# edwardyehuang/iSeg

Hardware: AMD Instinct MI355X
Metric: train_images_per_sec (ConvNeXt-T+ASPP 512x512 crop, fwd+bwd+AdamW, whole job) (higher is better)
Workload: dtype bf16

## Files before the change

include/iseg_hip.h:

```cpp
#ifndef ISEG_HIP_H
#define ISEG_HIP_H

#include <stddef.h>
#include <stdint.h>

#ifdef __cplusplus
extern "C" {
#endif

#ifndef ISEG_HIP_STREAM_T
#define ISEG_HIP_STREAM_T
typedef struct ihipStream_t* iseg_stream_t;
#endif

#define ISEG_STATUS_OK 0
#define ISEG_STATUS_ARG (-1)
#define ISEG_STATUS_HIP (-2)
#define ISEG_STATUS_UNSUPPORTED (-3)
#define ISEG_STATUS_WORKSPACE (-4)

#define ISEG_DTYPE_F32 0
#define ISEG_DTYPE_BF16 1

#define ISEG_ACT_NONE 0
// ... 46 lines not shown
int iseg_gemm_splits(const iseg_gemm_args* args_h);
int iseg_gemm_slabs(const iseg_gemm_args* args_h);
int iseg_gemm_variant(const iseg_gemm_args* args_h);
size_t iseg_gemm_workspace_bytes(const iseg_gemm_args* args_h);
int iseg_gemm(const iseg_gemm_args* args_h, void* ws, size_t ws_bytes, iseg_stream_t stream);
int iseg_gemm_reduce(const iseg_gemm_args* args_h, void* ws, size_t ws_bytes, iseg_stream_t stream);
int iseg_gemm_tn_pair_splits(const iseg_gemm_args* g0, const iseg_gemm_args* g1);
int iseg_gemm_tn_pair(const iseg_gemm_args* g0, void* ws0, size_t ws0_bytes, const iseg_gemm_args* g1, void* ws1, size_t ws1_bytes,
                      iseg_stream_t stream);

int iseg_layernorm_fwd(const void* x, const float* gamma, const float* beta, void* y, float* mean, float* rstd, int64_t rows,
                       int C, float eps, int dtype, iseg_stream_t stream);
size_t iseg_layernorm_bwd_workspace_bytes(int64_t rows, int C);
int iseg_layernorm_bwd(const void* dy, const void* x, const float* gamma, const float* mean, const float* rstd, void* dx,
                       const void* dx_add, float* dgamma, float* dbeta, int accumulate_param_grads, int64_t rows, int C,
                       int dtype, void* ws, size_t ws_bytes, iseg_stream_t stream);
int iseg_layernorm_post_fwd(const void* x, const float* gamma, const float* beta, const float* colscale, const float* rowscale,
                            int64_t rows_per_group, const void* residual, void* y, float* mean, float* rstd, int64_t rows, int C, float eps,
                            int dtype, iseg_stream_t stream);
int iseg_layernorm_post_bwd(const void* dy, const void* x, const float* gamma, const float* beta, const float* colscale, const float* rowscale,
                            int64_t rows_per_group, const float* mean, const float* rstd, void* dx, float* dgamma, float* dbeta,
                            float* dcolscale, int64_t rows, int C, int dtype, void* ws, size_t ws_bytes, iseg_stream_t stream);
int iseg_layernorm_gather_fwd(const void* x, const int32_t* src_index, const float* gamma, const float* beta, void* y, float* mean,
                              float* rstd, int64_t rows_out, int C, float eps, int dtype, iseg_stream_t stream);
int iseg_layernorm_gather_bwd(const void* dy, const int32_t* dy_index, const void* x, const float* gamma, const float* mean,
                              const float* rstd, void* dx, const void* dx_add, float* dgamma, float* dbeta, int accumulate_param_grads,
                              int64_t rows, int C, int dtype, void* ws, size_t ws_bytes, iseg_stream_t stream);

int iseg_dwconv2d_fwd(const void* x, const float* w, const float* bias, const void* add, void* y, int N, int H, int W, int C,
                      int K, int dil, int pad_t, int pad_l, int flip, int dtype, iseg_stream_t stream);
int iseg_dwconv2d7_mfma(const void* x, const float* w, const float* bias, const void* add, void* y, int N, int H, int W, int C, int pad_t,
                        int pad_l, int flip, iseg_stream_t stream);
size_t iseg_dwconv2d_bwd_weight_workspace_bytes(int N, int H, int W, int C, int K);
int iseg_dwconv2d_bwd_weight(const void* x, const void* dy, float* dw, float* db, int accumulate, int N, int H, int W, int C,
                             int K, int dil, int pad_t, int pad_l, int dtype, void* ws, size_t ws_bytes, iseg_stream_t stream);

int iseg_dwconv2d_strided_fwd(const void* x, const float* w, const float* bias, void* y, int N, int H, int W, int C, int K, int stride, int dil,
                              int pad_t, int pad_l, int Ho, int Wo, int dtype, iseg_stream_t stream);
int iseg_dwconv2d_strided_bwd_data(const void* dy, const float* w, void* dx, int N, int H, int W, int C, int K, int stride, int dil, int pad_t,
                                   int pad_l, int Ho, int Wo, int dtype, iseg_stream_t stream);
size_t iseg_dwconv2d_strided_bwd_weight_workspace_bytes(int N, int Ho, int Wo, int C, int K);
int iseg_dwconv2d_strided_bwd_weight(const void* x, const void* dy, float* dw, float* db, int accumulate, int N, int H, int W, int C, int K,
                                     int stride, int dil, int pad_t, int pad_l, int Ho, int Wo, int dtype, void* ws, size_t ws_bytes,
                                     iseg_stream_t stream);

size_t iseg_bn_workspace_bytes(int64_t rows, int C);
int iseg_bn_stats(const void* x, int64_t ldx, float* packed, int64_t rows, int C, int dtype, void* ws, size_t ws_bytes,
                  iseg_stream_t stream);
int iseg_bn_finalize(const float* packed, int C, float eps, float momentum, float* mean, float* rstd, float* moving_mean,
                     float* moving_var, iseg_stream_t stream);
int iseg_bn_apply_fwd(const void* x, int64_t ldx, const float* mean, const float* rstd, const float* gamma, const float* beta,
                      void* y, int64_t ldy, int64_t rows, int C, int relu, int dtype, iseg_stream_t stream);
int iseg_bn_apply_fwd_packed(const void* x, int64_t ldx, const float* packed, float eps, float momentum, const float* gamma, const float* beta,
                             float* mean, float* rstd, float* moving_mean, float* moving_var, void* y, int64_t ldy, int64_t rows, int C,
                             int relu, int dtype, iseg_stream_t stream);
int iseg_bn_bwd_reduce(const void* dy, int64_t lddy, const void* x, int64_t ldx, const void* y, int64_t ldy, const float* mean,
                       const float* rstd, float* sums, int64_t rows, int C, int relu, int dtype, void* ws, size_t ws_bytes,
                       iseg_stream_t stream);
int iseg_bn_bwd_apply(const void* dy, int64_t lddy, const void* x, int64_t ldx, const void* y, int64_t ldy, const float* mean,
                      const float* rstd, const float* gamma, const float* sums, float inv_n, void* dx, int64_t lddx, int64_t rows,
                      int C, int relu, int dtype, iseg_stream_t stream);
int iseg_bn_bwd_apply_acc(const void* dy, int64_t lddy, const void* x, int64_t ldx, const void* y, int64_t ldy, const float* mean,
                          const float* rstd, const float* gamma, const float* sums, float inv_n, void* dx, int64_t lddx, float* dgamma,
                          float* dbeta, int64_t rows, int C, int relu, int dtype, iseg_stream_t stream);
int iseg_bn_bwd_reduce_remask(const void* dy, int64_t lddy, const void* x, int64_t ldx, const float* mean, const float* rstd,
                              const float* gamma, const float* beta, float* sums, int64_t rows, int C, int dtype, void* ws, size_t ws_bytes,
// ... 348 lines not shown
```

iseg_amd/_hip.py:

```python
import ctypes as C
import os

_HERE = os.path.dirname(os.path.abspath(__file__))
LIB_PATH = os.path.join(_HERE, "lib", "libiseg_hip.so")

F32, BF16 = 0, 1
ACT_NONE, ACT_RELU, ACT_GELU, ACT_GELU_GRAD, ACT_RELU_GRAD, ACT_MUL_AUX, ACT_SIGMOID, ACT_SWISH = 0, 1, 2, 3, 4, 5, 6, 7


class HipLibraryMissing(RuntimeError):
    pass


class HipCallError(RuntimeError):
    pass


class GemmArgs(C.Structure):
    _fields_ = [
        ("A", C.c_void_p), ("lda", C.c_int64), ("a_kcontig", C.c_int),
        ("B", C.c_void_p), ("ldb", C.c_int64), ("b_kcontig", C.c_int),
        ("D", C.c_void_p), ("ldd", C.c_int64),
        ("M", C.c_int64), ("N", C.c_int64), ("K", C.c_int64),
        ("in_dtype", C.c_int), ("out_dtype", C.c_int),
# ... 16 lines not shown
    _fields_ = [(n, C.c_int) for n in ("N", "H", "W", "Cin", "Cout", "KH", "KW", "sh", "sw", "dh", "dw", "pt", "pl", "Ho", "Wo", "groups")]


_p, _i, _l, _f, _z, _u64 = C.c_void_p, C.c_int, C.c_int64, C.c_float, C.c_size_t, C.c_uint64

SIGNATURES = {
    "iseg_version": (_i, []),
    "iseg_last_error": (_z, [C.c_char_p, _z]),
    "iseg_gemm_splits": (_i, [C.POINTER(GemmArgs)]),
    "iseg_gemm_tn_pair_splits": (_i, [C.POINTER(GemmArgs), C.POINTER(GemmArgs)]),
    "iseg_gemm_tn_pair": (_i, [C.POINTER(GemmArgs), _p, _z, C.POINTER(GemmArgs), _p, _z, _p]),
    "iseg_gemm_slabs": (_i, [C.POINTER(GemmArgs)]),
    "iseg_gemm_variant": (_i, [C.POINTER(GemmArgs)]),
    "iseg_gemm_workspace_bytes": (_z, [C.POINTER(GemmArgs)]),
    "iseg_gemm": (_i, [C.POINTER(GemmArgs), _p, _z, _p]),
    "iseg_gemm_reduce": (_i, [C.POINTER(GemmArgs), _p, _z, _p]),
    "iseg_layernorm_fwd": (_i, [_p, _p, _p, _p, _p, _p, _l, _i, _f, _i, _p]),
    "iseg_layernorm_bwd_workspace_bytes": (_z, [_l, _i]),
    "iseg_layernorm_bwd": (_i, [_p, _p, _p, _p, _p, _p, _p, _p, _p, _i, _l, _i, _i, _p, _z, _p]),
    "iseg_layernorm_post_fwd": (_i, [_p, _p, _p, _p, _p, _l, _p, _p, _p, _p, _l, _i, _f, _i, _p]),
    "iseg_layernorm_post_bwd": (_i, [_p, _p, _p, _p, _p, _p, _l, _p, _p, _p, _p, _p, _p, _l, _i, _i, _p, _z, _p]),
    "iseg_layernorm_gather_fwd": (_i, [_p, _p, _p, _p, _p, _p, _p, _l, _i, _f, _i, _p]),
    "iseg_layernorm_gather_bwd": (_i, [_p, _p, _p, _p, _p, _p, _p, _p, _p, _p, _i, _l, _i, _i, _p, _z, _p]),
    "iseg_dwconv2d_fwd": (_i, [_p, _p, _p, _p, _p, _i, _i, _i, _i, _i, _i, _i, _i, _i, _i, _p]),
    "iseg_dcnv2_sample_fwd": (_i, [_p, _p, _p, _i, _i, _i, _i, _i, _p]),
    "iseg_dcnv2_sample_bwd_workspace_bytes": (_z, [_i, _i, _i, _i]),
    "iseg_dcnv2_sample_bwd": (_i, [_p, _p, _p, _p, _p, _i, _i, _i, _i, _i, _p, _z, _p]),
    "iseg_qkv_rope": (_i, [_p, _p, _p, _p, _p, _l, _i, _i, _i, _i, _i, _i, _p]),
    "iseg_glu_fwd": (_i, [_p, _l, _p, _l, _p, _l, _l, _i, _i, _i, _p]),
    "iseg_glu_bwd": (_i, [_p, _l, _p, _l, _p, _l, _p, _l, _p, _l, _l, _i, _i, _i, _p]),
    "iseg_dwconv2d7_mfma": (_i, [_p, _p, _p, _p, _p, _i, _i, _i, _i, _i, _i, _i, _p]),
    "iseg_dwconv2d_bwd_weight_workspace_bytes": (_z, [_i, _i, _i, _i, _i]),
    "iseg_dwconv2d_bwd_weight": (_i, [_p, _p, _p, _p, _i, _i, _i, _i, _i, _i, _i, _i, _i, _i, _p, _z, _p]),
    "iseg_dwconv2d_strided_fwd": (_i, [_p, _p, _p, _p, _i, _i, _i, _i, _i, _i, _i, _i, _i, _i, _i, _i, _p]),
    "iseg_dwconv2d_strided_bwd_data": (_i, [_p, _p, _p, _i, _i, _i, _i, _i, _i, _i, _i, _i, _i, _i, _i, _p]),
    "iseg_dwconv2d_strided_bwd_weight_workspace_bytes": (_z, [_i, _i, _i, _i, _i]),
    "iseg_dwconv2d_strided_bwd_weight": (_i, [_p, _p, _p, _p, _i, _i, _i, _i, _i, _i, _i, _i, _i, _i, _i, _i, _i, _p, _z, _p]),
    "iseg_dcn_center_blend_fwd": (_i, [_p, _p, _p, _p, _l, _i, _i, _i, _p]),
    "iseg_dcn_center_blend_bwd": (_i, [_p, _p, _p, _p, _p, _p, _p, _l, _i, _i, _i, _p]),
    "iseg_bn_workspace_bytes": (_z, [_l, _i]),
    "iseg_bn_stats": (_i, [_p, _l, _p, _l, _i, _i, _p, _z, _p]),
    "iseg_bn_finalize": (_i, [_p, _i, _f, _f, _p, _p, _p, _p, _p]),
    "iseg_bn_apply_fwd": (_i, [_p, _l, _p, _p, _p, _p, _p, _l, _l, _i, _i, _i, _p]),
    "iseg_bn_apply_fwd_packed": (_i, [_p, _l, _p, _f, _f, _p, _p, _p, _p, _p, _p, _p, _l, _l, _i, _i, _i, _p]),
    "iseg_bn_bwd_reduce": (_i, [_p, _l, _p, _l, _p, _l, _p, _p, _p, _l, _i, _i, _i, _p, _z, _p]),
    "iseg_bn_bwd_apply": (_i, [_p, _l, _p, _l, _p, _l, _p, _p, _p, _p, _f, _p, _l, _l, _i, _i, _i, _p]),
    "iseg_bn_bwd_apply_acc": (_i, [_p, _l, _p, _l, _p, _l, _p, _p, _p, _p, _f, _p, _l, _p, _p, _l, _i, _i, _i, _p]),
    "iseg_bn_bwd_reduce_remask": (_i, [_p, _l, _p, _l, _p, _p, _p, _p, _p, _l, _i, _i, _p, _z, _p]),
    "iseg_bn_bwd_apply_remask": (_i, [_p, _l, _p, _l, _p, _p, _p, _p, _p, _f, _p, _l, _p, _p, _l, _i, _i, _p]),
    "iseg_bn_relu_upsample_add": (_i, [_p, _p, _p, _p, _p, _p, _p, _i, _i, _i, _i, _i, _i, _i, _p]),
    "iseg_rsqrt_eps": (_i, [_p, _f, _p, _i, _p]),
    "iseg_mbconv_supported": (_i, [_i, _i, _i, _i]),
    "iseg_mbconv_partials_bytes": (_z, [_i, _i, _i, _i]),
    "iseg_se_excite_bwd_workspace_bytes": (_z, [_i, _i, _i]),
    "iseg_bn_swish_se_squeeze": (_i, [_p, _p, _p, _p, _p, _p, _z, _i, _i, _i, _i, _p]),
    "iseg_se_excite_fwd": (_i, [_p, _i, _i, _i, _i, _p, _p, _p, _p, _p, _p, _p, _p]),
    "iseg_bn_swish_gate_fwd": (_i, [_p, _p, _p, _p, _p, _p, _p, _i, _i, _i, _i, _p]),
    "iseg_bn_swish_gate_bwd_reduce": (_i, [_p, _p, _p, _p, _p, _p, _p, _z, _i, _i, _i, _i, _p]),
    "iseg_se_excite_bwd": (_i, [_p, _i, _i, _i, _i, _p, _p, _p, _p, _p, _p, _p, _p, _p, _i, _p, _p, _p, _z, _p]),
    "iseg_bn_swish_gate_bwd_apply": (_i, [_p, _p, _p, _p, _p, _p, _p, _p, _p, _f, _i, _p, _p, _p, _i, _i, _i, _i, _p]),
    "iseg_sepconv_supported": (_i, [_i, _i, _i, _i, _i, _i, _i]),
    "iseg_relu_dwconv3_stats_workspace_bytes": (_z, [_i, _i, _i, _i, _i, _i]),
    "iseg_relu_dwconv3_stats": (_i, [_p, _p, _p, _p, _i, _i, _i, _i, _i, _i, _i, _p, _z, _p]),
    "iseg_sepconv_fold": (_i, [_p, _p, _p, _p, _p, _p, _p, _p, _i, _i, _i, _p]),
    "iseg_sepconv_fold_bwd": (_i, [_p, _p, _p, _p, _p, _p, _p, _p, _p, _p, _p, _i, _i, _p]),
    "iseg_bnfold_dwconv3_relu_bwd_workspace_bytes": (_z, [_i, _i, _i, _i, _i, _i]),
# ... 178 lines not shown
```

iseg_amd/build.py:

```python
import os
import subprocess
import sys
from concurrent.futures import ThreadPoolExecutor

HERE = os.path.dirname(os.path.abspath(__file__))
ROOT = os.path.dirname(HERE)
CSRC = os.path.join(HERE, "csrc")
LIBDIR = os.path.join(HERE, "lib")
LIB = os.path.join(LIBDIR, "libiseg_hip.so")
SOURCES = ["api.hip", "gemm.hip", "gemm_nn.hip", "gemm_nt.hip", "gemm_tn.hip", "norm.hip", "dwconv.hip", "dwconv_mfma.hip", "dwconv_strided.hip", "elementwise.hip", "resize.hip", "loss.hip", "mask_loss.hip", "sod_metrics.hip", "sod_fmv2.hip", "optim.hip", "misc.hip", "attention.hip", "dcnv3.hip", "winattn.hip", "flashattn.hip", "mlp_fused.hip", "mlp_wgrad.hip", "conv_igemm.hip", "augment.hip", "grn.hip", "eva.hip", "comm.hip", "mbconv.hip", "sepconv.hip", "resblock.hip"]
FLAGS = ["--offload-arch=gfx950", "-O3", "-fPIC", "-std=c++17", "-I" + os.path.join(ROOT, "include"), "-I" + CSRC,
         "-Wno-unused-result"] + [f"-D{d}" for d in os.environ.get("ISEG_BUILD_DEFINES", "").split() if d]


def _hipcc():
    for c in (os.environ.get("HIPCC"), "/opt/rocm/bin/hipcc", "hipcc"):
        if c and (os.path.isabs(c) and os.path.exists(c) or not os.path.isabs(c)):
            return c
    raise RuntimeError("hipcc not found")


def _stale(out, deps):
    if not os.path.exists(out):
        return True
    t = os.path.getmtime(out)
    return any(os.path.getmtime(d) > t for d in deps)


def build(force=False, verbose=True):
    os.makedirs(LIBDIR, exist_ok=True)
    hipcc = _hipcc()
    headers = sorted(os.path.join(CSRC, f) for f in os.listdir(CSRC) if f.endswith(".h")) + [os.path.join(ROOT, "include", "iseg_hip.h")]
    objs, jobs = [], []
    for s in SOURCES:
        src = os.path.join(CSRC, s)
        obj = os.path.join(LIBDIR, s.replace(".hip", ".o"))
        objs.append(obj)
        if force or _stale(obj, [src] + headers):
            jobs.append([hipcc] + FLAGS + ["-c", src, "-o", obj])

    def run(cmd):
        if verbose:
            print(" ".join(cmd), flush=True)
# ... 16 lines not shown
```

iseg_amd/csrc/dwconv.hip:

```cpp
#include "common.h"
#include "iseg_hip.h"

namespace {

constexpr int TW = 4;
constexpr int BWSEG = 32;

template <class T, int CV> __device__ __forceinline__ void loadv(const T* p, float* out);
template <> __device__ __forceinline__ void loadv<float, 8>(const float* p, float* out) { load8<float>(p, out); }
template <> __device__ __forceinline__ void loadv<bf16_t, 8>(const bf16_t* p, float* out) { load8<bf16_t>(p, out); }
template <> __device__ __forceinline__ void loadv<float, 4>(const float* p, float* out) { Vec16<float>::load(p, out); }
template <> __device__ __forceinline__ void loadv<bf16_t, 4>(const bf16_t* p, float* out) {
    bf16x4 v = *reinterpret_cast<const bf16x4*>(p);
#pragma unroll
    for (int i = 0; i < 4; ++i) out[i] = (float)v[i];
}
template <class T, int CV> __device__ __forceinline__ void storev(T* p, const float* in);
template <> __device__ __forceinline__ void storev<float, 8>(float* p, const float* in) { store8<float>(p, in); }
template <> __device__ __forceinline__ void storev<bf16_t, 8>(bf16_t* p, const float* in) { store8<bf16_t>(p, in); }

static inline int groups_per_slab(int C, int CV, int maxg) {
    const int G = C / CV;
    int best = 1;
    for (int g = 1; g <= maxg && g <= G; ++g)
// ... 978 lines not shown
    const size_t lds = (size_t)g.rt * (K * K + 1) * g.gs * CV * sizeof(float);
    if (dil == 1)
        hipLaunchKernelGGL((dwconv_bwd_weight_kernel<T, K, CV, true>), dim3(g.bx, g.slabs), dim3(256), lds, s, (const T*)x,
                           (const T*)dy, ws, N, H, W, C, dil, pad_t, pad_l, g.gs, g.rt, g.wseg, g.ipl);
    else
        hipLaunchKernelGGL((dwconv_bwd_weight_kernel<T, K, CV, false>), dim3(g.bx, g.slabs), dim3(256), lds, s, (const T*)x,
                           (const T*)dy, ws, N, H, W, C, dil, pad_t, pad_l, g.gs, g.rt, g.wseg, g.ipl);
}

}

bool iseg_dwconv7_mfma_launch(const void* x, const float* w, const float* bias, const void* add, void* y, int N, int H, int W, int C, int K, int dil,
                              int pad_t, int pad_l, int flip, hipStream_t s);

extern "C" int iseg_dwconv2d_fwd(const void* x, const float* w, const float* bias, const void* add, void* y, int N, int H, int W,
                                 int C, int K, int dil, int pad_t, int pad_l, int flip, int dtype, hipStream_t stream) {
    ISEG_REQUIRE(x && w && y, "iseg_dwconv2d_fwd: null pointer");
    ISEG_REQUIRE(N > 0 && H > 0 && W > 0 && C > 0 && C % 8 == 0, "iseg_dwconv2d_fwd: C=%d must be a multiple of 8", C);
    ISEG_REQUIRE(K == 3 || K == 5 || K == 7, "iseg_dwconv2d_fwd: kernel size %d unsupported (3,5,7)", K);
    ISEG_REQUIRE(dil >= 1, "iseg_dwconv2d_fwd: dilation must be >= 1");
    ISEG_REQUIRE((int64_t)N * H * W * C < (1ll << 31), "iseg_dwconv2d_fwd: more than 2^31 elements");
#define DW_FWD(T)                                                                                             \
    (K == 7   ? launch_fwd_cv<T, 7>(x, w, bias, add, y, N, H, W, C, dil, pad_t, pad_l, flip, stream)          \
     : K == 5 ? launch_fwd_cv<T, 5>(x, w, bias, add, y, N, H, W, C, dil, pad_t, pad_l, flip, stream)          \
              : launch_fwd_cv<T, 3>(x, w, bias, add, y, N, H, W, C, dil, pad_t, pad_l, flip, stream))
    if (dtype == ISEG_BF16 && iseg_dwconv7_mfma_launch(x, w, bias, add, y, N, H, W, C, K, dil, pad_t, pad_l, flip, stream))
        return iseg_check_launch("iseg_dwconv2d (mfma)");
    if (dtype == ISEG_BF16 && launch_fwd_dma(x, w, bias, add, y, N, H, W, C, K, dil, pad_t, pad_l, flip, stream))
        return iseg_check_launch("iseg_dwconv2d");
    return dtype == ISEG_BF16 ? DW_FWD(bf16_t) : DW_FWD(float);
#undef DW_FWD
}

extern "C" size_t iseg_dwconv2d_bwd_weight_workspace_bytes(int N, int H, int W, int C, int K) {
    const BwGeom g = bw_geom(N, H, W, C, K, 1, 4);
    const BwGeom g2 = bw_geom(N, H, W, C, K, 2, 4);
    const BwGeom g3 = bw_geom(N, H, W, C, K, 1, 2);
    int bx = g.bx > g2.bx ? g.bx : g2.bx;
    if (g3.bx > bx) bx = g3.bx;
    const BwDmaGeom gd = bw_dma_geom(N, H, W, C, K, 1, 2);
    if (gd.ok && gd.bx > bx) bx = gd.bx;
    return (size_t)bx * (K * K + 1) * C * sizeof(float);
}

extern "C" int iseg_dwconv2d_bwd_weight(const void* x, const void* dy, float* dw, float* db, int accumulate, int N, int H, int W,
                                        int C, int K, int dil, int pad_t, int pad_l, int dtype, void* ws, size_t ws_bytes,
                                        hipStream_t stream) {
    ISEG_REQUIRE(x && dy && dw, "iseg_dwconv2d_bwd_weight: null pointer");
    ISEG_REQUIRE(C % 8 == 0, "iseg_dwconv2d_bwd_weight: C=%d must be a multiple of 8", C);
    ISEG_REQUIRE(K == 3 || K == 5 || K == 7, "iseg_dwconv2d_bwd_weight: kernel size %d unsupported", K);
    ISEG_REQUIRE((int64_t)N * H * W * C < (1ll << 31), "iseg_dwconv2d_bwd_weight: more than 2^31 elements");
    const BwDmaGeom gd = bw_dma_geom(N, H, W, C, K, dil, dtype == ISEG_BF16 ? 2 : 4);
    BwGeom g = bw_geom(N, H, W, C, K, dil, dtype == ISEG_BF16 ? 2 : 4);
    ISEG_REQUIRE(g.gs * K * g.rt <= 256, "iseg_dwconv2d_bwd_weight: slab does not fit a block");
    if (gd.ok) g.bx = gd.bx;
    const size_t need = (size_t)g.bx * (K * K + 1) * C * sizeof(float);
    if (!ws || ws_bytes < need) {
        iseg_set_error("iseg_dwconv2d_bwd_weight: needs %zu workspace bytes, got %zu", need, ws_bytes);
        return ISEG_ERR_WORKSPACE;
    }
    float* const arena = iseg_deferred_partials(need, dw, db, accumulate, stream);
    if (arena) ws = arena;
    if (gd.ok) {
        launch_bw_dma(x, dy, (float*)ws, N, H, W, C, pad_t, pad_l, gd, stream);
    } else if (g.lds) {
#define DW_BWL(KK)                                                                                                                   \
    hipLaunchKernelGGL((dwconv_bwd_weight_lds_kernel<float, KK>), dim3(g.bx, g.slabs), dim3(256), g.lds_bytes, stream, (const float*)x, \
                       (const float*)dy, (float*)ws, N, H, W, C, pad_t, pad_l, g.gs, g.rt, g.tiles_h, g.tiles_w)
        if (K == 7) DW_BWL(7);
        else if (K == 5) DW_BWL(5);
        else DW_BWL(3);
#undef DW_BWL
    } else if (dtype == ISEG_BF16) {
        if (K == 7) launch_bw<bf16_t, 7>(x, dy, (float*)ws, N, H, W, C, dil, pad_t, pad_l, g, stream);
        else if (K == 5) launch_bw<bf16_t, 5>(x, dy, (float*)ws, N, H, W, C, dil, pad_t, pad_l, g, stream);
        else launch_bw<bf16_t, 3>(x, dy, (float*)ws, N, H, W, C, dil, pad_t, pad_l, g, stream);
    } else {
        if (K == 7) launch_bw<float, 7>(x, dy, (float*)ws, N, H, W, C, dil, pad_t, pad_l, g, stream);
        else if (K == 5) launch_bw<float, 5>(x, dy, (float*)ws, N, H, W, C, dil, pad_t, pad_l, g, stream);
        else launch_bw<float, 3>(x, dy, (float*)ws, N, H, W, C, dil, pad_t, pad_l, g, stream);
    }
    const int n = (K * K + 1) * C;
    if (arena) iseg_deferred_push((const float*)ws, g.bx, n, n, dw, db, K * K * C, 1.f, stream);
    else launch_reduce_rows((const float*)ws, g.bx, n, 0, 1, n, dw, db, K * K * C, 0, 1.f, accumulate, stream);
    return iseg_check_launch("iseg_dwconv2d_bwd_weight");
}
```

iseg_amd/csrc/dwconv_mfma.hip:

```cpp
#include "common.h"
#include "iseg_hip.h"

namespace {

typedef __attribute__((ext_vector_type(4))) short s16x4;
typedef __attribute__((ext_vector_type(4))) float f32x4_t;
typedef __attribute__((address_space(3))) void* dwm_lds_ptr;
typedef const __attribute__((address_space(1))) void* dwm_glb_ptr;

__device__ uint4 dwm_zero_page[4];

constexpr int TR = 16, TC = 16, CH = 32, KS = 7, WAVES = 8;
constexpr int RAW_ROWS = TR + 8, RAW_COLS = TC + 6, RAW_PITCH = 23;
constexpr int RAW_PIXELS = RAW_ROWS * RAW_PITCH, RAW_PIECES = (RAW_PIXELS + 15) / 16;
constexpr int NPW = (RAW_PIECES + WAVES - 1) / WAVES;
constexpr int RAW_BUF = NPW * WAVES * 1024;
constexpr int PLANE = 1248, COLP = 56;
constexpr int P_BYTES = CH * PLANE;
constexpr int O_PITCH = TC * CH * 4 + 64;
constexpr int O_BYTES = TR * O_PITCH;
constexpr int P_OFF = 2 * RAW_BUF, O_OFF = P_OFF + P_BYTES, LDS_BYTES = O_OFF + O_BYTES;
static_assert(RAW_COLS * COLP <= PLANE && LDS_BYTES <= 160 * 1024, "one workgroup of 8 wavefronts per CU");

typedef __attribute__((ext_vector_type(2))) unsigned u32x2_t;
typedef __attribute__((ext_vector_type(4))) unsigned u32x4_t;

#define DWM_BARRIER()                                       \
    do {                                                    \
        asm volatile("s_waitcnt lgkmcnt(0)" ::: "memory"); \
        __builtin_amdgcn_s_barrier();                       \
        asm volatile("" ::: "memory");                      \
    } while (0)
#define DWM_GUARD7(N, A)                                                                                                                        \
    asm volatile("s_waitcnt lgkmcnt(%7)" : "+v"((A)[0]), "+v"((A)[1]), "+v"((A)[2]), "+v"((A)[3]), "+v"((A)[4]), "+v"((A)[5]), "+v"((A)[6]) \
                 : "n"(N) : "memory")

__global__ __launch_bounds__(64 * WAVES) void dwconv7_mfma_kernel(const bf16_t* __restrict__ x, const float* __restrict__ w,
                                                                const float* __restrict__ bias, const bf16_t* __restrict__ add,
                                                                bf16_t* __restrict__ y, int N, int H, int W, int C, int pad_t, int pad_l, int flip,
                                                                int tiles_h, int tiles_w, int slabs, int units_per_wg) {
    extern __shared__ __attribute__((aligned(1024))) char smem_dwm[];
    const unsigned lds0 = (unsigned)(uintptr_t)(dwm_lds_ptr)smem_dwm;
    const int tid = threadIdx.x, lane = tid & 63, wid = __builtin_amdgcn_readfirstlane(tid >> 6);
    const int ntiles = N * tiles_h * tiles_w, units = ntiles * slabs;
    int lb = blockIdx.x;
    if (gridDim.x % 8 == 0) lb = (blockIdx.x % 8) * (gridDim.x / 8) + blockIdx.x / 8;
    const int u_begin = lb * units_per_wg, u_end = min(units, u_begin + units_per_wg);
    if (u_begin >= u_end) return;

    int prc[NPW];
#pragma unroll
    for (int i = 0; i < NPW; ++i) {
        const int pix = (wid + WAVES * i) * 16 + (lane >> 2);
        const int rr = pix / RAW_PITCH, cc = pix - rr * RAW_PITCH;
        prc[i] = (cc >= RAW_COLS || rr >= TR + KS - 1) ? -1 : (rr << 16) | cc;
    }
    const bf16_t* const zero = reinterpret_cast<const bf16_t*>(dwm_zero_page) + (lane & 3) * 8;
    const int tg = lane >> 4, ti = lane & 15;
    const unsigned tr_src = lds0 + (((ti >> 2) * RAW_PITCH) + (tg >> 1)) * 64 + (tg & 1) * 32 + (ti & 3) * 8;
    const unsigned tr_dst = lds0 + P_OFF + ((tg & 1) * 16 + ti) * PLANE + (tg >> 1) * COLP;
    const int chg = wid & 1, strip = wid >> 1, chl = lane >> 2, mn = lane & 3;
    const unsigned frag_base = lds0 + P_OFF + (chg * 16 + chl) * PLANE + (mn + 4 * strip) * COLP;
    const unsigned out_base = lds0 + O_OFF + mn * O_PITCH + (4 * strip) * (CH * 4) + (chg * 16 + chl) * 4;

    unsigned t_src[9], t_dst[9];
// ... 247 lines not shown
```

iseg_amd/kernels.py:

```python
import contextlib
import ctypes as C

import torch

from . import _hip
from ._hip import F32, BF16, ACT_NONE, ACT_RELU, ACT_GELU, ACT_GELU_GRAD, ACT_RELU_GRAD, ACT_MUL_AUX, ACT_SIGMOID, ACT_SWISH, GemmArgs

_DT = {torch.float32: F32, torch.bfloat16: BF16}


def dt(t):
    try:
        return _DT[t.dtype if isinstance(t, torch.Tensor) else t]
    except KeyError:
        raise TypeError(f"iseg_amd kernels support float32 and bfloat16 storage, got {t.dtype if isinstance(t, torch.Tensor) else t}")


def ptr(t):
    return None if t is None else t.data_ptr()


_DEVICE_INDEX = [None]


# ... 614 lines not shown
    return dz2, dsc


def dwconv2d(x, w, bias, K, dil, pad_t, pad_l, *, flip=False, add=None):
    _require_cuda(x)
    N, H, W, Cc = x.shape
    y = torch.empty_like(x)
    timer = KERNEL_TIMER[0]
    if timer is not None:
        timer.begin(("dwconv", int(N), int(H), int(W), int(Cc), int(K), int(dil), bool(flip), add is not None, x.dtype))
    _hip.call("iseg_dwconv2d_fwd", ptr(x), ptr(w), ptr(bias), ptr(add), ptr(y), N, H, W, Cc, K, dil, pad_t, pad_l, int(flip), dt(x),
              stream())
    if timer is not None:
        timer.end()
    return y


def dwconv2d7_mfma(x, w, bias, pad_t=3, pad_l=3, *, flip=False, add=None):
    _require_cuda(x)
    N, H, W, Cc = x.shape
    y = torch.empty_like(x)
    _hip.call("iseg_dwconv2d7_mfma", ptr(x), ptr(w), ptr(bias), ptr(add), ptr(y), N, H, W, Cc, pad_t, pad_l, int(flip), stream())
    return y


def dwconv2d_bwd_weight(x, dy, dw, db, K, dil, pad_t, pad_l, accumulate=True):
    N, H, W, Cc = x.shape
    need = _hip.lib().iseg_dwconv2d_bwd_weight_workspace_bytes(N, H, W, Cc, K)
    ws, wsb = workspace(need, x.device)
    _hip.call("iseg_dwconv2d_bwd_weight", ptr(x), ptr(dy), ptr(dw), ptr(db), int(accumulate), N, H, W, Cc, K, dil, pad_t, pad_l,
              dt(x), ptr(ws), wsb, stream())


def dwconv2d_strided(x, w, bias, K, stride, dil):
    _require_cuda(x, w)
    N, H, W, Cc = x.shape
    Ho, pt = same_pad(H, K, stride, dil)
    Wo, pl = same_pad(W, K, stride, dil)
    y = torch.empty((N, Ho, Wo, Cc), dtype=x.dtype, device=x.device)
    _hip.call("iseg_dwconv2d_strided_fwd", ptr(x), ptr(w), ptr(bias), ptr(y), N, H, W, Cc, K, stride, dil, pt, pl, Ho, Wo, dt(x), stream())
    return y


def dwconv2d_strided_bwd_data(dy, w, K, stride, dil, H, W):
    _require_cuda(dy, w)
    N, Ho, Wo, Cc = dy.shape
    _, pt = same_pad(H, K, stride, dil)
    _, pl = same_pad(W, K, stride, dil)
    dx = torch.empty((N, H, W, Cc), dtype=dy.dtype, device=dy.device)
    _hip.call("iseg_dwconv2d_strided_bwd_data", ptr(dy), ptr(w), ptr(dx), N, H, W, Cc, K, stride, dil, pt, pl, Ho, Wo, dt(dy), stream())
    return dx


def dwconv2d_strided_bwd_weight(x, dy, dw, db, K, stride, dil, accumulate=True):
    _require_cuda(x, dy, dw)
    N, H, W, Cc = x.shape
    _, Ho, Wo, _ = dy.shape
    _, pt = same_pad(H, K, stride, dil)
    _, pl = same_pad(W, K, stride, dil)
    need = _hip.lib().iseg_dwconv2d_strided_bwd_weight_workspace_bytes(N, Ho, Wo, Cc, K)
    ws, wsb = workspace(need, x.device)
    _hip.call("iseg_dwconv2d_strided_bwd_weight", ptr(x), ptr(dy), ptr(dw), ptr(db), int(accumulate), N, H, W, Cc, K, stride, dil, pt, pl, Ho, Wo,
              dt(x), ptr(ws), wsb, stream())


def cast(src, dst_dtype, out=None):
# ... 926 lines not shown
```

Measured before the change: 1965.

## Add matrix-core weight-gradient kernel for 7x7 depthwise conv and auto-dispatch it

Adds a new kernel that computes the 7x7 depthwise convolution weight and bias gradients with 4x4x4 bf16 MFMA instructions. It stages x and dy tiles into LDS by DMA, transposes them with ds_read_b64_tr_b16, and double-buffers the next tile's loads behind the matrix work. The generic bwd_weight entry now routes to this kernel for bf16 inputs when they are aligned, C is a multiple of 32 and the problem is large enough. The aim is to replace the scalar/VALU reduction path with matrix-core accumulation. In exchange it adds a larger workspace sizing rule and a complex new LDS layout, and changes the order of floating-point summation.

New measurement: 2007, median of 6. 2.1% higher.

```diff
diff --git a/include/iseg_hip.h b/include/iseg_hip.h
--- a/include/iseg_hip.h
+++ b/include/iseg_hip.h
@@ -102,6 +102,8 @@
 int iseg_dwconv2d7_mfma(const void* x, const float* w, const float* bias, const void* add, void* y, int N, int H, int W, int C, int pad_t,
                         int pad_l, int flip, iseg_stream_t stream);
 size_t iseg_dwconv2d_bwd_weight_workspace_bytes(int N, int H, int W, int C, int K);
+int iseg_dwconv2d7_bwd_weight_mfma(const void* x, const void* dy, float* dw, float* db, int accumulate, int N, int H, int W, int C, int pad_t,
+                                   int pad_l, void* ws, size_t ws_bytes, iseg_stream_t stream);
 int iseg_dwconv2d_bwd_weight(const void* x, const void* dy, float* dw, float* db, int accumulate, int N, int H, int W, int C,
                              int K, int dil, int pad_t, int pad_l, int dtype, void* ws, size_t ws_bytes, iseg_stream_t stream);
 
diff --git a/iseg_amd/_hip.py b/iseg_amd/_hip.py
--- a/iseg_amd/_hip.py
+++ b/iseg_amd/_hip.py
@@ -72,6 +72,7 @@
     "iseg_dwconv2d7_mfma": (_i, [_p, _p, _p, _p, _p, _i, _i, _i, _i, _i, _i, _i, _p]),
     "iseg_dwconv2d_bwd_weight_workspace_bytes": (_z, [_i, _i, _i, _i, _i]),
     "iseg_dwconv2d_bwd_weight": (_i, [_p, _p, _p, _p, _i, _i, _i, _i, _i, _i, _i, _i, _i, _i, _p, _z, _p]),
+    "iseg_dwconv2d7_bwd_weight_mfma": (_i, [_p, _p, _p, _p, _i, _i, _i, _i, _i, _i, _i, _p, _z, _p]),
     "iseg_dwconv2d_strided_fwd": (_i, [_p, _p, _p, _p, _i, _i, _i, _i, _i, _i, _i, _i, _i, _i, _i, _i, _p]),
     "iseg_dwconv2d_strided_bwd_data": (_i, [_p, _p, _p, _i, _i, _i, _i, _i, _i, _i, _i, _i, _i, _i, _i, _p]),
     "iseg_dwconv2d_strided_bwd_weight_workspace_bytes": (_z, [_i, _i, _i, _i, _i]),
diff --git a/iseg_amd/build.py b/iseg_amd/build.py
--- a/iseg_amd/build.py
+++ b/iseg_amd/build.py
@@ -8,7 +8,7 @@
 CSRC = os.path.join(HERE, "csrc")
 LIBDIR = os.path.join(HERE, "lib")
 LIB = os.path.join(LIBDIR, "libiseg_hip.so")
-SOURCES = ["api.hip", "gemm.hip", "gemm_nn.hip", "gemm_nt.hip", "gemm_tn.hip", "norm.hip", "dwconv.hip", "dwconv_mfma.hip", "dwconv_strided.hip", "elementwise.hip", "resize.hip", "loss.hip", "mask_loss.hip", "sod_metrics.hip", "sod_fmv2.hip", "optim.hip", "misc.hip", "attention.hip", "dcnv3.hip", "winattn.hip", "flashattn.hip", "mlp_fused.hip", "mlp_wgrad.hip", "conv_igemm.hip", "augment.hip", "grn.hip", "eva.hip", "comm.hip", "mbconv.hip", "sepconv.hip", "resblock.hip"]
+SOURCES = ["api.hip", "gemm.hip", "gemm_nn.hip", "gemm_nt.hip", "gemm_tn.hip", "norm.hip", "dwconv.hip", "dwconv_mfma.hip", "dwconv_wgrad_mfma.hip", "dwconv_strided.hip", "elementwise.hip", "resize.hip", "loss.hip", "mask_loss.hip", "sod_metrics.hip", "sod_fmv2.hip", "optim.hip", "misc.hip", "attention.hip", "dcnv3.hip", "winattn.hip", "flashattn.hip", "mlp_fused.hip", "mlp_wgrad.hip", "conv_igemm.hip", "augment.hip", "grn.hip", "eva.hip", "comm.hip", "mbconv.hip", "sepconv.hip", "resblock.hip"]
 FLAGS = ["--offload-arch=gfx950", "-O3", "-fPIC", "-std=c++17", "-I" + os.path.join(ROOT, "include"), "-I" + CSRC,
          "-Wno-unused-result"] + [f"-D{d}" for d in os.environ.get("ISEG_BUILD_DEFINES", "").split() if d]
 
diff --git a/iseg_amd/csrc/dwconv.hip b/iseg_amd/csrc/dwconv.hip
--- a/iseg_amd/csrc/dwconv.hip
+++ b/iseg_amd/csrc/dwconv.hip
@@ -1034,6 +1034,16 @@
 #undef DW_FWD
 }
 
+int iseg_dwconv7_wgrad_mfma_blocks(int N, int H, int W, int C, int K, int dil);
+bool iseg_dwconv7_wgrad_mfma_launch(const void* x, const void* dy, float* partials, int N, int H, int W, int C, int pad_t, int pad_l, int blocks,
+                                    hipStream_t s);
+
+static bool bw_mfma_auto(const void* x, const void* dy, int N, int H, int W, int C) {
+    if ((((uintptr_t)x | (uintptr_t)dy) & 15) != 0 || C % 32 != 0) return false;
+    const int64_t units = (int64_t)N * ((H + 15) / 16) * ((W + 15) / 16) * (C / 16);
+    return units >= 768;
+}
+
 extern "C" size_t iseg_dwconv2d_bwd_weight_workspace_bytes(int N, int H, int W, int C, int K) {
     const BwGeom g = bw_geom(N, H, W, C, K, 1, 4);
     const BwGeom g2 = bw_geom(N, H, W, C, K, 2, 4);
@@ -1042,6 +1052,8 @@
     if (g3.bx > bx) bx = g3.bx;
     const BwDmaGeom gd = bw_dma_geom(N, H, W, C, K, 1, 2);
     if (gd.ok && gd.bx > bx) bx = gd.bx;
+    const int bm = iseg_dwconv7_wgrad_mfma_blocks(N, H, W, C, K, 1);
+    if (bm > bx) bx = bm;
     return (size_t)bx * (K * K + 1) * C * sizeof(float);
 }
 
@@ -1056,6 +1068,8 @@
     BwGeom g = bw_geom(N, H, W, C, K, dil, dtype == ISEG_BF16 ? 2 : 4);
     ISEG_REQUIRE(g.gs * K * g.rt <= 256, "iseg_dwconv2d_bwd_weight: slab does not fit a block");
     if (gd.ok) g.bx = gd.bx;
+    const int bm = dtype == ISEG_BF16 && bw_mfma_auto(x, dy, N, H, W, C) ? iseg_dwconv7_wgrad_mfma_blocks(N, H, W, C, K, dil) : 0;
+    if (bm) g.bx = bm;
     const size_t need = (size_t)g.bx * (K * K + 1) * C * sizeof(float);
     if (!ws || ws_bytes < need) {
         iseg_set_error("iseg_dwconv2d_bwd_weight: needs %zu workspace bytes, got %zu", need, ws_bytes);
@@ -1063,7 +1077,12 @@
     }
     float* const arena = iseg_deferred_partials(need, dw, db, accumulate, stream);
     if (arena) ws = arena;
-    if (gd.ok) {
+    if (bm) {
+        if (!iseg_dwconv7_wgrad_mfma_launch(x, dy, (float*)ws, N, H, W, C, pad_t, pad_l, bm, stream)) {
+            iseg_set_error("iseg_dwconv2d_bwd_weight: the matrix-core kernel could not be launched");
+            return ISEG_ERR_UNSUPPORTED;
+        }
+    } else if (gd.ok) {
         launch_bw_dma(x, dy, (float*)ws, N, H, W, C, pad_t, pad_l, gd, stream);
     } else if (g.lds) {
 #define DW_BWL(KK)                                                                                                                   \
diff --git a/iseg_amd/csrc/dwconv_mfma.hip b/iseg_amd/csrc/dwconv_mfma.hip
--- a/iseg_amd/csrc/dwconv_mfma.hip
+++ b/iseg_amd/csrc/dwconv_mfma.hip
@@ -1,12 +1,15 @@
 #include "common.h"
+#include "dwconv_mfma_common.h"
 #include "iseg_hip.h"
 
 namespace {
 
-typedef __attribute__((ext_vector_type(4))) short s16x4;
-typedef __attribute__((ext_vector_type(4))) float f32x4_t;
-typedef __attribute__((address_space(3))) void* dwm_lds_ptr;
-typedef const __attribute__((address_space(1))) void* dwm_glb_ptr;
+using dwm::s16x4;
+using dwm::f32x4_t;
+using dwm::u32x2_t;
+using dwm::u32x4_t;
+typedef dwm::lds_ptr dwm_lds_ptr;
+typedef dwm::glb_ptr dwm_glb_ptr;
 
 __device__ uint4 dwm_zero_page[4];
 
@@ -22,15 +25,6 @@
 constexpr int P_OFF = 2 * RAW_BUF, O_OFF = P_OFF + P_BYTES, LDS_BYTES = O_OFF + O_BYTES;
 static_assert(RAW_COLS * COLP <= PLANE && LDS_BYTES <= 160 * 1024, "one workgroup of 8 wavefronts per CU");
 
-typedef __attribute__((ext_vector_type(2))) unsigned u32x2_t;
-typedef __attribute__((ext_vector_type(4))) unsigned u32x4_t;
-
-#define DWM_BARRIER()                                       \
-    do {                                                    \
-        asm volatile("s_waitcnt lgkmcnt(0)" ::: "memory"); \
-        __builtin_amdgcn_s_barrier();                       \
-        asm volatile("" ::: "memory");                      \
-    } while (0)
 #define DWM_GUARD7(N, A)                                                                                                                        \
     asm volatile("s_waitcnt lgkmcnt(%7)" : "+v"((A)[0]), "+v"((A)[1]), "+v"((A)[2]), "+v"((A)[3]), "+v"((A)[4]), "+v"((A)[5]), "+v"((A)[6]) \
                  : "n"(N) : "memory")
diff --git a/iseg_amd/csrc/dwconv_mfma_common.h b/iseg_amd/csrc/dwconv_mfma_common.h
--- /dev/null
+++ b/iseg_amd/csrc/dwconv_mfma_common.h
@@ -0,0 +1,24 @@
+#pragma once
+#include "common.h"
+
+namespace dwm {
+
+typedef __attribute__((ext_vector_type(4))) short s16x4;
+typedef __attribute__((ext_vector_type(4))) float f32x4_t;
+typedef __attribute__((ext_vector_type(2))) unsigned u32x2_t;
+typedef __attribute__((ext_vector_type(4))) unsigned u32x4_t;
+typedef __attribute__((address_space(3))) void* lds_ptr;
+typedef const __attribute__((address_space(1))) void* glb_ptr;
+
+__device__ __forceinline__ void lds_read_tr16_b64(u32x2_t& out, unsigned addr) {
+    asm volatile("ds_read_b64_tr_b16 %0, %1" : "=v"(out) : "v"(addr) : "memory");
+}
+
+}
+
+#define DWM_BARRIER()                                       \
+    do {                                                    \
+        asm volatile("s_waitcnt lgkmcnt(0)" ::: "memory"); \
+        __builtin_amdgcn_s_barrier();                       \
+        asm volatile("" ::: "memory");                      \
+    } while (0)
diff --git a/iseg_amd/csrc/dwconv_wgrad_mfma.hip b/iseg_amd/csrc/dwconv_wgrad_mfma.hip
--- /dev/null
+++ b/iseg_amd/csrc/dwconv_wgrad_mfma.hip
@@ -0,0 +1,267 @@
+#include "common.h"
+#include "dwconv_mfma_common.h"
+#include "iseg_hip.h"
+
+namespace {
+
+using dwm::f32x4_t;
+using dwm::s16x4;
+using dwm::u32x2_t;
+
+__device__ uint4 wgm_zero_page[2];
+
+constexpr int TR = 16, TC = 16, CH = 16, KS = 7, NT = KS * KS + 1, WAVES = 4;
+constexpr int X_ROWS = 24, X_COLS = 22, X_PITCH = 22;
+constexpr int X_PIECES = (X_ROWS * X_PITCH + 31) / 32;
+constexpr int D_PITCH = 18, D_PIECES = TR * D_PITCH / 32;
+constexpr int D_TOP = 2048, D_BOT = 2048;
+static_assert(TR * D_PITCH % 32 == 0 && 3 * D_PITCH * 32 <= D_TOP && 2 * D_PITCH * 32 <= D_BOT, "dY tile layout");
+constexpr int PLANE = 1248, COLP = 56;
+constexpr int E_COL = 48, E_PLANE = TC * E_COL + 16, E_COPY = CH * E_PLANE + 128;
+constexpr int RX_OFF = 0, RD_OFF = RX_OFF + X_PIECES * 1024, PX_OFF = RD_OFF + D_TOP + D_PIECES * 1024 + D_BOT, PE_OFF = PX_OFF + CH * PLANE;
+constexpr int LDS_BYTES = PE_OFF + 2 * E_COPY;
+constexpr int X_TASKS = 6 * 6, E_TASKS = 2 * 5 * 4;
+constexpr int NPX = (X_PIECES + WAVES - 1) / WAVES, NPD = (D_PIECES + WAVES - 1) / WAVES;
+static_assert(X_COLS * COLP <= PLANE && LDS_BYTES <= 80 * 1024 && PX_OFF % 8 == 0 && PE_OFF % 8 == 0, "two workgroups per CU");
+static_assert(WAVES * NT * CH * 4 + WAVES * 4 * CH * 4 <= LDS_BYTES, "final reduction fits");
+
+template <int QI>
+__device__ __forceinline__ void wgm_column(unsigned a_base, unsigned b_base, f32x4_t (&acc)[2][2]) {
+    u32x2_t a[2][6], b[5];
+#define WGM_RDA(G, CK) asm volatile("ds_read_b64 %0, %1 offset:%2" : "=v"(a[G][CK]) : "v"(a_base), "n"((QI + 4 * (G)) * COLP + (CK) * 8) : "memory")
+#define WGM_RDB(J) \
+    asm volatile("ds_read2_b32 %0, %1 offset0:%2 offset1:%3" : "=v"(b[J]) : "v"(b_base), "n"(QI * (E_COL / 4) + 2 * (J)), "n"(QI * (E_COL / 4) + 2 * (J) + 1) : "memory")
+    WGM_RDB(0); WGM_RDA(0, 0); WGM_RDA(1, 0); WGM_RDA(0, 1); WGM_RDA(1, 1);
+    WGM_RDB(1); WGM_RDA(0, 2); WGM_RDA(1, 2);
+    WGM_RDB(2); WGM_RDA(0, 3); WGM_RDA(1, 3);
+    WGM_RDB(3); WGM_RDA(0, 4); WGM_RDA(1, 4);
+    WGM_RDB(4); WGM_RDA(0, 5); WGM_RDA(1, 5);
+#undef WGM_RDA
+#undef WGM_RDB
+    asm volatile("s_waitcnt lgkmcnt(0)" : "+v"(a[0][0]), "+v"(a[0][1]), "+v"(a[0][2]), "+v"(a[0][3]), "+v"(a[0][4]), "+v"(a[0][5]), "+v"(a[1][0]),
+                 "+v"(a[1][1]), "+v"(a[1][2]), "+v"(a[1][3]), "+v"(a[1][4]), "+v"(a[1][5]), "+v"(b[0]), "+v"(b[1]), "+v"(b[2]), "+v"(b[3]), "+v"(b[4])
+                 :: "memory");
+#pragma unroll
+    for (int j = 0; j < 5; ++j) {
+        const s16x4 bj = __builtin_bit_cast(s16x4, b[j]);
+#pragma unroll
+        for (int g = 0; g < 2; ++g) {
+            acc[0][g] = __builtin_amdgcn_mfma_f32_4x4x4bf16_1k(__builtin_bit_cast(s16x4, a[g][j]), bj, acc[0][g], 0, 0, 0);
+            acc[1][g] = __builtin_amdgcn_mfma_f32_4x4x4bf16_1k(__builtin_bit_cast(s16x4, a[g][j + 1]), bj, acc[1][g], 0, 0, 0);
+        }
+    }
+}
+
+__global__ __launch_bounds__(64 * WAVES, 2) void dwconv7_wgrad_mfma_kernel(const bf16_t* __restrict__ x, const bf16_t* __restrict__ dy,
+                                                                          float* __restrict__ partials, int N, int H, int W, int C, int pad_t,
+                                                                          int pad_l, int tiles_h, int tiles_w, int tiles_per_wg) {
+    extern __shared__ __attribute__((aligned(1024))) char smem_wgm[];
+    const unsigned lds0 = (unsigned)(uintptr_t)(dwm::lds_ptr)smem_wgm;
+    const int tid = threadIdx.x, lane = tid & 63, wid = __builtin_amdgcn_readfirstlane(tid >> 6);
+    const int c0 = blockIdx.y * CH;
+    const int ntiles = N * tiles_h * tiles_w;
+    int lb = blockIdx.x;
+    if (gridDim.x % 8 == 0) lb = (blockIdx.x % 8) * (gridDim.x / 8) + blockIdx.x / 8;
+    const int t_begin = min(ntiles, lb * tiles_per_wg), t_end = min(ntiles, t_begin + tiles_per_wg);
+
+    for (int i = tid; i < (D_TOP + D_BOT) / 8; i += 64 * WAVES) {
+        const int o = i * 8 < D_TOP ? i * 8 : D_TOP + D_PIECES * 1024 + (i * 8 - D_TOP);
+        *reinterpret_cast<uint2*>(smem_wgm + RD_OFF + o) = make_uint2(0u, 0u);
+    }
+    for (int i = tid; i < 2 * CH * TC; i += 64 * WAVES) {
+        const int s = i / (CH * TC), ch = (i / TC) % CH, col = i % TC;
+        *reinterpret_cast<uint2*>(smem_wgm + PE_OFF + s * E_COPY + ch * E_PLANE + col * E_COL + 40) = make_uint2(0u, 0u);
+    }
+
+    int xrc[NPX], drc[NPD];
+#pragma unroll
+    for (int i = 0; i < NPX; ++i) {
+        const int pix = (wid + WAVES * i) * 32 + (lane >> 1);
+        const int rr = pix / X_PITCH, cc = pix - rr * X_PITCH;
+        xrc[i] = ((rr >= TR + KS - 1 ? 0x7fff : rr) << 16) | cc;
+    }
+#pragma unroll
+    for (int i = 0; i < NPD; ++i) {
+        const int pix = (wid + WAVES * i) * 32 + (lane >> 1);
+        const int rr = pix / D_PITCH, cc = pix - rr * D_PITCH;
+        drc[i] = ((cc >= TC || rr >= TR ? 0x7fff : rr) << 16) | cc;
+    }
+    const bf16_t* const zero = reinterpret_cast<const bf16_t*>(wgm_zero_page) + (lane & 1) * 8;
+    auto issue_dma = [&](int tile) {
+        int b = tile;
+        const int tw_i = b % tiles_w;
+        b /= tiles_w;
+        const int th_i = b % tiles_h;
+        const int n = b / tiles_h;
+        const int h0 = th_i * TR, w0 = tw_i * TC;
+        const bf16_t* xb = x + (((n * H + h0 - pad_t) * W + w0 - pad_l) * C + c0 + (lane & 1) * 8);
+        const bf16_t* db = dy + (((n * H + h0) * W + w0) * C + c0 + (lane & 1) * 8);
+#pragma unroll
+        for (int i = 0; i < NPX; ++i) {
+            const int p = wid + WAVES * i;
+            if (p < X_PIECES) {
+                int rc = xrc[i];
+                asm volatile("" : "+v"(rc));
+                const int rr = rc >> 16, cc = rc & 0xffff;
+                const bool ok = (unsigned)(h0 - pad_t + rr) < (unsigned)H && (unsigned)(w0 - pad_l + cc) < (unsigned)W;
+                const bf16_t* src = ok ? xb + __mul24(__mul24(rr, W) + cc, C) : zero;
+                __builtin_amdgcn_global_load_lds((dwm::glb_ptr)src, (dwm::lds_ptr)(smem_wgm + RX_OFF + p * 1024), 16, 0, 0);
+            }
+        }
+#pragma unroll
+        for (int i = 0; i < NPD; ++i) {
+            const int p = wid + WAVES * i;
+            if (p < D_PIECES) {
+                int rc = drc[i];
+                asm volatile("" : "+v"(rc));
+                const int rr = rc >> 16, cc = rc & 0xffff;
+                const bool ok = (unsigned)(h0 + rr) < (unsigned)H && (unsigned)(w0 + cc) < (unsigned)W;
+                const bf16_t* src = ok ? db + __mul24(__mul24(rr, W) + cc, C) : zero;
+                __builtin_amdgcn_global_load_lds((dwm::glb_ptr)src, (dwm::lds_ptr)(smem_wgm + RD_OFF + D_TOP + p * 1024), 16, 0, 0);
+            }
+        }
+    };
+    const int tg = lane >> 4, ti = lane & 15;
+    const unsigned trx_src = lds0 + RX_OFF + (((ti >> 2) * X_PITCH) + tg) * 32 + (ti & 3) * 8;
+    const unsigned trx_dst = lds0 + PX_OFF + ti * PLANE + tg * COLP;
+    const unsigned trd_src = lds0 + RD_OFF + D_TOP + (((ti >> 2) * D_PITCH) + tg) * 32 + (ti & 3) * 8;
+    const unsigned trd_dst = lds0 + PE_OFF + ti * E_PLANE + tg * E_COL;
+    const int chl = lane >> 2, mn = lane & 3;
+    const unsigned a_base = lds0 + PX_OFF + chl * PLANE + (4 * wid + mn) * COLP;
+    const unsigned b_base = lds0 + PE_OFF + (mn & 1) * E_COPY + chl * E_PLANE + (4 * wid) * E_COL + 4 - 4 * (mn >> 1);
+
+    f32x4_t acc[2][2];
+#pragma unroll
+    for (int i = 0; i < 2; ++i)
+#pragma unroll
+        for (int j = 0; j < 2; ++j) acc[i][j] = f32x4_t{0.f, 0.f, 0.f, 0.f};
+    float accb = 0.f;
+
+    if (t_begin < t_end) issue_dma(t_begin);
+    for (int tile = t_begin; tile < t_end; ++tile) {
+        asm volatile("s_waitcnt vmcnt(0)" ::: "memory");
+        __syncthreads();
+
+        {
+            u32x2_t tv[9] = {};
+#pragma unroll
+            for (int i = 0; i < 9; ++i) {
+                const int task = wid + WAVES * i, R = task / 6, cq = task - R * 6;
+                dwm::lds_read_tr16_b64(tv[i], trx_src + (4 * R * X_PITCH + 4 * cq) * 32);
+            }
+            asm volatile("s_waitcnt lgkmcnt(0)" : "+v"(tv[0]), "+v"(tv[1]), "+v"(tv[2]), "+v"(tv[3]), "+v"(tv[4]), "+v"(tv[5]), "+v"(tv[6]), "+v"(tv[7]), "+v"(tv[8])
+                         :: "memory");
+#pragma unroll
+            for (int i = 0; i < 9; ++i) {
+                const int task = wid + WAVES * i, R = task / 6, cq = task - R * 6;
+                if (4 * cq + tg < X_COLS)
+                    asm volatile("ds_write_b64 %0, %1" ::"v"(trx_dst + (4 * cq) * COLP + R * 8), "v"(tv[i]) : "memory");
+            }
+        }
+        {
+            u32x2_t tv[10] = {};
+#pragma unroll
+            for (int i = 0; i < 10; ++i) {
+                const int task = wid + WAVES * i, s = task / 20, T = (task / 4) % 5, cq = task & 3;
+                dwm::lds_read_tr16_b64(tv[i], trd_src + ((4 * T - 2 - s) * D_PITCH + 4 * cq) * 32);
+            }
+            asm volatile("s_waitcnt lgkmcnt(0)" : "+v"(tv[0]), "+v"(tv[1]), "+v"(tv[2]), "+v"(tv[3]), "+v"(tv[4]), "+v"(tv[5]), "+v"(tv[6]), "+v"(tv[7]), "+v"(tv[8]),
+                         "+v"(tv[9]) :: "memory");
+#pragma unroll
+            for (int i = 0; i < 10; ++i) {
+                const int task = wid + WAVES * i, s = task / 20, T = (task / 4) % 5, cq = task & 3;
+                asm volatile("ds_write_b64 %0, %1" ::"v"(trd_dst + s * E_COPY + (4 * cq) * E_COL + T * 8), "v"(tv[i]) : "memory");
+                if (s == 0) {
+                    accb += __uint_as_float(tv[i].x << 16);
+                    accb += __uint_as_float(tv[i].x & 0xffff0000u);
+                    accb += __uint_as_float(tv[i].y << 16);
+                    accb += __uint_as_float(tv[i].y & 0xffff0000u);
+                }
+            }
+        }
+        DWM_BARRIER();
+
+        if (tile + 1 < t_end) issue_dma(tile + 1);
+
+        wgm_column<0>(a_base, b_base, acc);
+        wgm_column<1>(a_base, b_base, acc);
+        wgm_column<2>(a_base, b_base, acc);
+        wgm_column<3>(a_base, b_base, acc);
+    }
+    asm volatile("s_waitcnt vmcnt(0)" ::: "memory");
+    __syncthreads();
+
+    float* red = reinterpret_cast<float*>(smem_wgm);
+    float* redb = red + WAVES * (NT - 1) * CH;
+#pragma unroll
+    for (int kyg = 0; kyg < 2; ++kyg)
+#pragma unroll
+        for (int kxg = 0; kxg < 2; ++kxg)
+#pragma unroll
+            for (int m = 0; m < 4; ++m) {
+                const int ky = 4 * kyg + mn, kx = 4 * kxg + m;
+                if (ky < KS && kx < KS) red[(wid * (NT - 1) + ky * KS + kx) * CH + chl] = acc[kyg][kxg][m];
+            }
+    redb[(wid * 4 + tg) * CH + ti] = accb;
+    __syncthreads();
+    float* out = partials + (int64_t)blockIdx.x * NT * C;
+    for (int i = tid; i < NT * CH; i += 64 * WAVES) {
+        const int tap = i / CH, c = i % CH;
+        float s = 0.f;
+        if (tap < NT - 1) {
+            for (int w = 0; w < WAVES; ++w) s += red[(w * (NT - 1) + tap) * CH + c];
+        } else {
+            for (int w = 0; w < WAVES * 4; ++w) s += redb[w * CH + c];
+        }
+        out[(int64_t)tap * C + c0 + c] = s;
+    }
+}
+
+}
+
+int iseg_dwconv7_wgrad_mfma_blocks(int N, int H, int W, int C, int K, int dil) {
+    if (K != KS || dil != 1 || C % 32 != 0 || N <= 0 || H <= 0 || W <= 0) return 0;
+    const int64_t ntiles = (int64_t)N * ((H + TR - 1) / TR) * ((W + TC - 1) / TC);
+    if (ntiles >= (1ll << 30)) return 0;
+    int64_t cap = 512 / (C / CH);
+    if (cap < 8) cap = 8;
+    const int64_t rounds = ceil_div64(ntiles, cap);
+    int64_t bx = ceil_div64(ntiles, rounds);
+    if (bx % 8 && (bx + 7) / 8 * 8 <= ntiles) bx = (bx + 7) / 8 * 8;
+    return (int)bx;
+}
+
+bool iseg_dwconv7_wgrad_mfma_launch(const void* x, const void* dy, float* partials, int N, int H, int W, int C, int pad_t, int pad_l, int blocks,
+                                    hipStream_t s) {
+    if (blocks <= 0 || (((uintptr_t)x | (uintptr_t)dy) & 15) != 0) return false;
+    static const bool raised = [] {
+        return hipFuncSetAttribute(reinterpret_cast<const void*>(&dwconv7_wgrad_mfma_kernel), hipFuncAttributeMaxDynamicSharedMemorySize, LDS_BYTES) ==
+               hipSuccess;
+    }();
+    if (!raised) return false;
+    const int tiles_h = (H + TR - 1) / TR, tiles_w = (W + TC - 1) / TC;
+    const int64_t ntiles = (int64_t)N * tiles_h * tiles_w;
+    const int per = (int)ceil_div64(ntiles, blocks);
+    hipLaunchKernelGGL(dwconv7_wgrad_mfma_kernel, dim3((unsigned)blocks, C / CH), dim3(64 * WAVES), LDS_BYTES, s, (const bf16_t*)x, (const bf16_t*)dy,
+                       partials, N, H, W, C, pad_t, pad_l, tiles_h, tiles_w, per);
+    return true;
+}
+
+extern "C" int iseg_dwconv2d7_bwd_weight_mfma(const void* x, const void* dy, float* dw, float* db, int accumulate, int N, int H, int W, int C,
+                                              int pad_t, int pad_l, void* ws, size_t ws_bytes, hipStream_t stream) {
+    ISEG_REQUIRE(x && dy && dw && N > 0 && H > 0 && W > 0, "iseg_dwconv2d7_bwd_weight_mfma: bad arguments");
+    ISEG_REQUIRE((int64_t)N * H * W * C < (1ll << 31), "iseg_dwconv2d7_bwd_weight_mfma: more than 2^31 elements");
+    const int blocks = iseg_dwconv7_wgrad_mfma_blocks(N, H, W, C, KS, 1);
+    const size_t need = (size_t)blocks * NT * C * sizeof(float);
+    if (blocks > 0 && (!ws || ws_bytes < need)) {
+        iseg_set_error("iseg_dwconv2d7_bwd_weight_mfma: needs %zu workspace bytes, got %zu", need, ws_bytes);
+        return ISEG_ERR_WORKSPACE;
+    }
+    if (!iseg_dwconv7_wgrad_mfma_launch(x, dy, (float*)ws, N, H, W, C, pad_t, pad_l, blocks, stream)) {
+        iseg_set_error("iseg_dwconv2d7_bwd_weight_mfma: needs bf16 storage, C %% 32 == 0 (C = %d) and 16-byte aligned tensors", C);
+        return ISEG_ERR_UNSUPPORTED;
+    }
+    const int n = NT * C;
+    launch_reduce_rows((const float*)ws, blocks, n, 0, 1, n, dw, db, (int64_t)(NT - 1) * C, 0, 1.f, accumulate, stream);
+    return iseg_check_launch("iseg_dwconv2d7_bwd_weight_mfma");
+}
diff --git a/iseg_amd/kernels.py b/iseg_amd/kernels.py
--- a/iseg_amd/kernels.py
+++ b/iseg_amd/kernels.py
@@ -670,6 +670,14 @@
               dt(x), ptr(ws), wsb, stream())
 
 
+def dwconv2d7_bwd_weight_mfma(x, dy, dw, db, pad_t=3, pad_l=3, accumulate=True):
+    _require_cuda(x, dy, dw)
+    N, H, W, Cc = x.shape
+    need = _hip.lib().iseg_dwconv2d_bwd_weight_workspace_bytes(N, H, W, Cc, 7)
+    ws, wsb = workspace(need, x.device)
+    _hip.call("iseg_dwconv2d7_bwd_weight_mfma", ptr(x), ptr(dy), ptr(dw), ptr(db), int(accumulate), N, H, W, Cc, pad_t, pad_l, ptr(ws), wsb, stream())
+
+
 def dwconv2d_strided(x, w, bias, K, stride, dil):
     _require_cuda(x, w)
     N, H, W, Cc = x.shape
```
